# LabJunBMI/E3-invaraint-diffusion-model

Measured on AMD Instinct MI355X. Metric: denoising-steps/sec (batched pocket graphs), higher is better.
Workload: dtype f32 storage and accumulation, f16x3 products (fp32 grade); 1 GPU; structure_model sampling step, 256 x 256-residue pockets per GPU, 12+12 layers x 768, T=1000 schedule, encoder recomputed every step (as the reference); pockets_per_gpu=256, seq_len=256, parallelism=pocket-sharded x1, no collective

## Files before the change

### e3-invaraint-diffusion-model_amd/csrc/gemm_split.hip

```cpp
#include <type_traits>

#include "e3d_common.h"

namespace {

typedef __bf16 bf16x8 __attribute__((ext_vector_type(8)));
typedef __bf16 bf16x4 __attribute__((ext_vector_type(4)));
typedef _Float16 f16x8 __attribute__((ext_vector_type(8)));
typedef _Float16 f16x4 __attribute__((ext_vector_type(4)));

template <typename E> struct Vec;
template <> struct Vec<__bf16> { typedef bf16x8 x8; typedef bf16x4 x4; };
template <> struct Vec<_Float16> { typedef f16x8 x8; typedef f16x4 x4; };
__device__ __forceinline__ f32x16 mma16(const bf16x8 a, const bf16x8 b, const f32x16 c) {
    return __builtin_amdgcn_mfma_f32_32x32x16_bf16(a, b, c, 0, 0, 0);
}
__device__ __forceinline__ f32x16 mma16(const f16x8 a, const f16x8 b, const f32x16 c) {
    return __builtin_amdgcn_mfma_f32_32x32x16_f16(a, b, c, 0, 0, 0);
}

struct Epi { float* absmax; float scale; };

constexpr int BN = 128, BK = 32;
#ifdef GEMM_STAMPS
// ... 681 lines not shown
#pragma unroll
    for (int m = 0; m < 4; ++m) {
#pragma unroll
        for (int n = 0; n < 2; ++n) {
            const int col = col0 + wc * 64 + n * 32 + l31;
            const float bv = bias ? bias[col] : 0.f;
#pragma unroll
            for (int r = 0; r < 16; ++r) {
                const int row = row0 + wr * 128 + m * 32 + mfma32_row(r, half);
                float v = fmaf(acc[m][n][r], out_scale, bv);
                if (ACT == E3D_ACT_GELU) v = gelu_erf(v);
                if (ACT == E3D_ACT_SILU) v = silu(v);
                if (row < M) {
                    out[(int64_t)row * ldc + col] = v;
                    if (ACT == E3D_ACT_NONE && absmax) e3d_absmax_accum(amax, v);
                }
            }
        }
    }
    if (ACT == E3D_ACT_NONE && absmax) e3d_absmax_commit(amax, absmax, lane);
    STAMP_K(4);
#ifdef E3D_STAMPS
    asm volatile("s_waitcnt vmcnt(0)" ::: "memory");
    STAMP_K(5);
#endif
}

#ifdef E3D_NT_STORES
#define E3D_STORE_OUT(ptr, val) __builtin_nontemporal_store((val), (ptr))
#else
#define E3D_STORE_OUT(ptr, val) (*(ptr) = (val))
#endif

template <int ACT, typename E>
__global__ __launch_bounds__(512, 2) void gemm_split256p_kernel(const float* __restrict__ A, int64_t lda,
                                                                 const float* __restrict__ W,
                                                                 const float* __restrict__ bias,
                                                                 float* __restrict__ out, int64_t ldc, int N, int K,
                                                                 int tiles_m, int tiles_n, float* __restrict__ absmax, float out_scale) {
    extern __shared__ __attribute__((aligned(16))) unsigned char smem_raw[];
    constexpr int NS = 2, T_BYTES = BT * ROW64, BUF_BYTES = 2 * NS * T_BYTES;
    constexpr int NI = 8;
    const int total = tiles_m * tiles_n, nk = K / BK;
    const int tid = threadIdx.x, lane = tid & 63, wid = tid >> 6;
    const int wr = wid >> 2, wc = wid & 3;
    const int l31 = lane & 31, half = lane >> 5;

    unsigned goff[NI];
    int dst[NI];
#pragma unroll
    for (int i = 0; i < NI; ++i) {
        const int f = tid + 512 * (i & 3), r = f >> 3, kg = f & 7;
        goff[i] = (unsigned)(r * (i < 4 ? (int)lda : K) + kg * 4);
        dst[i] = (i < 4 ? 0 : NS * T_BYTES) + swz_off(r, kg >> 1) + (kg & 1) * 8;
    }

    int ld_tile = blockIdx.x, ld_k = 0;
    const float* ld_a;
    const float* ld_w;
    auto cursor_bases = [&]() {
        const int lid = xcd_remap(ld_tile, total);
        ld_a = A + (int64_t)(lid / tiles_n) * BT * lda + ld_k * BK;
        ld_w = W + (int64_t)(lid % tiles_n) * BT * K + ld_k * BK;
    };
    auto cursor_advance = [&]() {
        if (ld_k + 1 < nk) {
            ++ld_k;
            ld_a += BK;
            ld_w += BK;
        } else if (ld_tile + (int)gridDim.x < total) {
            ld_tile += gridDim.x;
            ld_k = 0;
            cursor_bases();
        }
    };
    f32x4 rg[NI];
    auto item_load = [&](int i) { rg[i] = *reinterpret_cast<const f32x4*>((i < 4 ? ld_a : ld_w) + goff[i]); };
    auto item_store = [&](int i, unsigned char* buf) {
        typename Vec<E>::x4 p[NS];
        split4<NS, E>(rg[i], p);
#pragma unroll
        for (int s = 0; s < NS; ++s) *reinterpret_cast<typename Vec<E>::x4*>(buf + s * T_BYTES + dst[i]) = p[s];
    };
    cursor_bases();
#pragma unroll
    for (int i = 0; i < NI; ++i) item_load(i);
    cursor_advance();
#pragma unroll
    for (int i = 0; i < NI; ++i) item_store(i, smem_raw);
#pragma unroll
    for (int i = 0; i < NI; ++i) item_load(i);
    cursor_advance();
    __syncthreads();

    int a_row[4], b_row[2];
#pragma unroll
    for (int m = 0; m < 4; ++m) a_row[m] = wr * 128 + m * 32 + l31;
#pragma unroll
    for (int n = 0; n < 2; ++n) b_row[n] = wc * 64 + n * 32 + l31;
    int cur = 0;
    unsigned amax = 0;

    for (int tile = blockIdx.x; tile < total; tile += gridDim.x) {
        f32x16 acc[4][2];
#pragma unroll
        for (int m = 0; m < 4; ++m)
#pragma unroll
            for (int n = 0; n < 2; ++n)
#pragma unroll
                for (int r = 0; r < 16; ++r) acc[m][n][r] = 0.f;
        for (int kt = 0; kt < nk; ++kt) {
            const unsigned char* base = smem_raw + cur * BUF_BYTES;
            unsigned char* next = smem_raw + (cur ^ 1) * BUF_BYTES;
#pragma unroll
            for (int ks = 0; ks < 2; ++ks) {
                typename Vec<E>::x8 fa[NS][4], fb[NS][2];
#pragma unroll
                for (int s = 0; s < NS; ++s) {
#pragma unroll
                    for (int n = 0; n < 2; ++n)
                        fb[s][n] = *reinterpret_cast<const typename Vec<E>::x8*>(base + (NS + s) * T_BYTES +
                                                                    swz_off(b_row[n], 2 * ks + half));
#pragma unroll
                    for (int m = 0; m < 4; ++m)
                        fa[s][m] = *reinterpret_cast<const typename Vec<E>::x8*>(base + s * T_BYTES + swz_off(a_row[m], 2 * ks + half));
                }
#pragma unroll
                for (int m = 0; m < 4; ++m) {
                    const int g = ks * 4 + m;
                    item_store(g, next);
                    item_load(g);
#pragma unroll
                    for (int n = 0; n < 2; ++n) {
                        acc[m][n] = mma16(fa[0][m], fb[1][n], acc[m][n]);
                        acc[m][n] = mma16(fa[1][m], fb[0][n], acc[m][n]);
                        acc[m][n] = mma16(fa[0][m], fb[0][n], acc[m][n]);
                    }
                    __builtin_amdgcn_sched_barrier(0);
                }
            }
            cursor_advance();
            __syncthreads();
            cur ^= 1;
        }

        const int lid = xcd_remap(tile, total);
        const int row0 = (lid / tiles_n) * BT, col0 = (lid % tiles_n) * BT;
#pragma unroll
        for (int m = 0; m < 4; ++m) {
#pragma unroll
            for (int n = 0; n < 2; ++n) {
                const int col = col0 + wc * 64 + n * 32 + l31;
                const float bv = bias ? bias[col] : 0.f;
                float* o = out + (int64_t)(row0 + wr * 128 + m * 32 + 4 * half) * ldc + col;
#pragma unroll
                for (int r = 0; r < 16; ++r) {
                    float v = fmaf(acc[m][n][r], out_scale, bv);
                    if (ACT == E3D_ACT_GELU) v = gelu_erf(v);
                    if (ACT == E3D_ACT_SILU) v = silu(v);
                    E3D_STORE_OUT(&o[(int64_t)((r & 3) + 8 * (r >> 2)) * ldc], v);
                    if (ACT == E3D_ACT_NONE && absmax) e3d_absmax_accum(amax, v);
                }
            }
        }
    }
    if (ACT == E3D_ACT_NONE && absmax) e3d_absmax_commit(amax, absmax, lane);
}

template <int ACT, typename E>
int launch256p(const float* A, int64_t lda, const float* W, const float* bias, float* out, int64_t ldc, int M, int N,
               int K, Epi epi, hipStream_t s) {
    const int tiles_m = M / BT, tiles_n = N / BT;
    constexpr size_t lds = 2 * 2 * 2 * BT * ROW64;
    static std::atomic<uint64_t> lds_ok{0};
    const int n_cu = e3d_cu_count();
    const int total = tiles_m * tiles_n;
    e3d_allow_lds(lds_ok, gemm_split256p_kernel<ACT, E>, lds);
    hipLaunchKernelGGL((gemm_split256p_kernel<ACT, E>), dim3(total < n_cu ? total : n_cu), dim3(512), lds, s, A, lda, W, bias, out,
                       ldc, N, K, tiles_m, tiles_n, epi.absmax, epi.scale);
    return e3d_launch_status("e3d_gemm_f32_split (persistent 256x256)");
}

int g_general_form = -1;
int g_tile_pref = -1;

template <int NS, int ACT, int WR, int WC, int NBUF, bool PIPE, typename E>
int launch256(const float* A, int64_t lda, const float* W, const float* bias, float* out, int64_t ldc, int M, int N,
              int K, Epi epi, hipStream_t s) {
    constexpr int TM = WR * 128, TN = WC * 64;
    const int tiles_m = (M + TM - 1) / TM, tiles_n = N / TN;
    const size_t lds = (size_t)NBUF * NS * (TM + TN) * ROW64;
    static std::atomic<uint64_t> lds_ok{0};
    e3d_allow_lds(lds_ok, gemm_split256_kernel<NS, ACT, WR, WC, NBUF, PIPE, E>, lds);
    hipLaunchKernelGGL((gemm_split256_kernel<NS, ACT, WR, WC, NBUF, PIPE, E>), dim3(tiles_m * tiles_n), dim3(WR * WC * 64), lds, s,
                       A, lda, W, bias, out, ldc, M, N, K, tiles_m, tiles_n, epi.absmax, epi.scale);
    return e3d_launch_status("e3d_gemm_f32_split (128x64 wave tiles)");
}

template <int NS, int ACT, bool A_KMAJ, bool B_KMAJ, int WM, int WN, typename E, int TN = 2, bool TR = false>
int launch_general(const float* A, int64_t lda, const float* B, int64_t ldb, const float* bias, float* out, int64_t ldc,
                   int M, int N, int K, Epi epi, hipStream_t s);

int p_min() {
    static int v = 0;
    if (!v) {
        const char* e = getenv("E3D_GEMM_P_MIN");
        v = e ? atoi(e) : 160;
    }
    return v;
}

template <int NS, int ACT, bool A_KMAJ, bool B_KMAJ, typename E>
int launch(const float* A, int64_t lda, const float* B, int64_t ldb, const float* bias, float* out, int64_t ldc,
           int M, int N, int K, Epi epi, hipStream_t s) {
    if (g_tile_pref < 0) {
        const char* e = getenv("E3D_GEMM_TILE");
        g_tile_pref = e ? atoi(e) : 4;
// ... 86 lines not shown
    return e3d_launch_status("e3d_gemm_f32_split");
}

template <int NS, typename E>
int dispatch(int act, bool a_kmaj, bool b_kmaj, const float* A, int64_t lda, const float* B, int64_t ldb,
             const float* bias, float* out, int64_t ldc, int M, int N, int K, Epi epi, hipStream_t s) {
    if (!a_kmaj && !b_kmaj) {
        switch (act) {
            case E3D_ACT_NONE: return launch<NS, E3D_ACT_NONE, false, false, E>(A, lda, B, ldb, bias, out, ldc, M, N, K, epi, s);
            case E3D_ACT_GELU: return launch<NS, E3D_ACT_GELU, false, false, E>(A, lda, B, ldb, bias, out, ldc, M, N, K, epi, s);
            case E3D_ACT_SILU: return launch<NS, E3D_ACT_SILU, false, false, E>(A, lda, B, ldb, bias, out, ldc, M, N, K, epi, s);
        }
        e3d_set_error("gemm_split: unknown activation %d", act);
        return -1;
    }
    if (act != E3D_ACT_NONE) {
        e3d_set_error("gemm_split: activations are only fused for the forward (K-contiguous) layout");
        return -1;
    }
    if (!a_kmaj && b_kmaj) return launch<NS, E3D_ACT_NONE, false, true, __bf16>(A, lda, B, ldb, bias, out, ldc, M, N, K, epi, s);
    if (a_kmaj && b_kmaj) return launch<NS, E3D_ACT_NONE, true, true, __bf16>(A, lda, B, ldb, bias, out, ldc, M, N, K, Epi{nullptr, epi.scale}, s);
    return launch<NS, E3D_ACT_NONE, true, false, __bf16>(A, lda, B, ldb, bias, out, ldc, M, N, K, epi, s);
}

}

#ifdef GEMM_STAMPS
extern "C" int e3d_debug_gemm_stamps(long long* t) { return (int)hipMemcpyFromSymbol(t, HIP_SYMBOL(gemm_stamps), sizeof(long long) * 2 * 64 * 8); }
#endif

#ifdef E3D_STAMPS
extern "C" int e3d_debug_read_stamps(long long* host_out) {
    return (int)hipMemcpyFromSymbol(host_out, HIP_SYMBOL(e3d_stamps), sizeof(long long) * 2 * 32 * 8);
}
#endif

extern "C" int e3d_gemm_kernel_select(int pref) {
    if (g_tile_pref < 0) {
        const char* e = getenv("E3D_GEMM_TILE");
        g_tile_pref = e ? atoi(e) : 4;
    }
    const int prev = g_tile_pref;
    if (pref >= 0) g_tile_pref = pref;
    return prev;
}

extern "C" int e3d_gemm_general_select(int form) {
    if (g_general_form < 0) {
        const char* e = getenv("E3D_GEMM_FORM");
        g_general_form = e ? atoi(e) : 0;
    }
    const int prev = g_general_form;
    if (form >= 0) g_general_form = form;
    return prev;
}

static int gemm_split_general(const float* A, int64_t lda, int a_kmajor, const float* B, int64_t ldb, int b_kmajor,
                              const float* bias, float* out, int64_t ldc, int M, int N, int K, int act, int terms,
                              float* absmax, float out_scale, void* stream) {
    const Epi epi{absmax, out_scale};
    E3D_REQUIRE(out_scale == 1.0f || !(a_kmajor && b_kmajor), "gemm_split: out_scale is not available for the split-K layout");
    E3D_REQUIRE(A && B && out, "gemm_split: null pointer");
    E3D_REQUIRE(M > 0 && N > 0 && K > 0, "gemm_split: bad shape M=%d N=%d K=%d", M, N, K);
    E3D_REQUIRE(terms == E3D_TERMS_BF16 || terms == 3 || terms == 6 || terms == E3D_TERMS_F16X3,
                "gemm_split: terms must be 1, 3, 6 or 19 (got %d)", terms);
    E3D_REQUIRE(ldc >= N, "gemm_split: ldc=%lld < N=%d", (long long)ldc, N);
// ... 134 lines not shown
```

### e3-invaraint-diffusion-model_amd/csrc/gemm_rowln.hip

```cpp
#include <type_traits>

#include "e3d_common.h"

namespace {

typedef __bf16 bf16x8 __attribute__((ext_vector_type(8)));
typedef _Float16 f16x8 __attribute__((ext_vector_type(8)));
template <typename E> struct V8;
template <> struct V8<__bf16> { typedef bf16x8 t; };
template <> struct V8<_Float16> { typedef f16x8 t; };
__device__ __forceinline__ f32x16 mma16(const bf16x8 a, const bf16x8 b, const f32x16 c) {
    return __builtin_amdgcn_mfma_f32_32x32x16_bf16(a, b, c, 0, 0, 0);
}
__device__ __forceinline__ f32x16 mma16(const f16x8 a, const f16x8 b, const f32x16 c) {
    return __builtin_amdgcn_mfma_f32_32x32x16_f16(a, b, c, 0, 0, 0);
}

constexpr int RN = 768, RBM = 96, NBLK = RN / 32;
constexpr int W_STEP = NBLK * 2 * 1024;
constexpr int A_PAIR = 128 * 128;
constexpr int LDS_A = 2 * W_STEP;
constexpr int RES_CHUNK = 16 * RN * 4;
constexpr int LDS_STATS = 3 * RES_CHUNK;
constexpr int LDS_COLS = LDS_STATS + (8 * RBM + RBM) * 4;
// ... 27 lines not shown
    const int piece = blockIdx.x * 4 + (threadIdx.x >> 6);
    const int nblk = N / 32;
    if (piece >= (K / 16) * nblk) return;
    const int ks = piece / nblk, nb = piece % nblk;
    const float* src = W + (int64_t)(nb * 32 + (lane & 31)) * K + ks * 16 + 8 * (lane >> 5);
    const f32x4 a = *reinterpret_cast<const f32x4*>(src), b = *reinterpret_cast<const f32x4*>(src + 4);
    typename V8<E>::t hi, lo;
    split8(a, b, hi, lo);
    unsigned char* dst = out + (int64_t)piece * 2048 + lane * 16;
    *reinterpret_cast<typename V8<E>::t*>(dst) = hi;
    *reinterpret_cast<typename V8<E>::t*>(dst + 1024) = lo;
}

#ifndef ROWLN_LAB
#define ROWLN_LAB 0
#endif
#ifdef ROWLN_STAMPS
__device__ long long rowln_stamps[2][64][8];
__device__ long long rowln_tile_stamps[2][8][8];
__device__ long long rowln_wg_times[512][4];
#define RSTAMP(step, slot)                                                                                        \
    do {                                                                                                          \
        if (stamp_on && (step) < 64 && lane == 0) rowln_stamps[wid >> 2][(step)][(slot)] = __builtin_readcyclecounter(); \
    } while (0)
#define TSTAMP(slot)                                                                                              \
    do {                                                                                                          \
        if (stamp_on && tile_no < 8 && lane == 0) rowln_tile_stamps[wid >> 2][tile_no][(slot)] = __builtin_readcyclecounter(); \
    } while (0)
#else
#define RSTAMP(step, slot) do {} while (0)
#define TSTAMP(slot) do {} while (0)
#endif
#define E3D_VMCNT(n) asm volatile("s_waitcnt vmcnt(" #n ")" ::: "memory")
#define E3D_BARRIER()                          \
    do {                                       \
        asm volatile("" ::: "memory");         \
        __builtin_amdgcn_s_barrier();          \
        asm volatile("" ::: "memory");         \
        __builtin_amdgcn_sched_barrier(0);     \
    } while (0)
#define E3D_LDS_BARRIER()                                   \
    do {                                                    \
        asm volatile("s_waitcnt lgkmcnt(0)" ::: "memory");  \
        E3D_BARRIER();                                      \
    } while (0)

template <int OFF = 0>
__device__ __forceinline__ void glds16(const void* g, unsigned char* lds_wave_base) {
    __builtin_amdgcn_global_load_lds((const __attribute__((address_space(1))) void*)g,
                                     (__attribute__((address_space(3))) void*)lds_wave_base, 16, OFF, 0);
}

__device__ __forceinline__ int next_tile_rows(int left, int pattern, int group_rows) {
#ifndef ROWLN_NO_PATTERNS
    if (group_rows == 256) {
        if (pattern == 1 && left == 256) return 64;
        if (pattern == 2 && left == 160) return 64;
        if (pattern == 3) return 64;
    }
#endif
    if (left >= 160 || left == 96) return 96;
    if (left > 96) return 64;
    return left;
}

template <typename E>
__global__ __launch_bounds__(512, 2) void gemm_rowln_kernel(const float* __restrict__ A, int64_t lda,
                                                            const unsigned char* __restrict__ Wp, const float* __restrict__ bias,
                                                            const float* __restrict__ res, int64_t ldr,
                                                            const float* __restrict__ gamma, const float* __restrict__ beta,
                                                            float eps, float* __restrict__ out, int64_t ldo, int M, int K,
                                                            int rows_per_wg, float out_scale) {
    extern __shared__ __attribute__((aligned(16))) unsigned char smem[];
    typedef typename V8<E>::t X8;
    const int tid = threadIdx.x, lane = tid & 63;
    const int wid = __builtin_amdgcn_readfirstlane(tid >> 6);
    const int l31 = lane & 31, half = lane >> 5;
    const int npairs = K / 32, last_step = 2 * npairs - 1;

    int row0 = blockIdx.x * rows_per_wg;
    const int row_end = min(M, row0 + rows_per_wg);
    if (row0 >= row_end) return;

    const unsigned w_lane = (unsigned)(wid * 6144 + lane * 16);
    unsigned a_lane[2];
    auto a_offsets = [&](int rows) {
#pragma unroll
        for (int i = 0; i < 2; ++i) {
            const int row = (wid + 8 * i) * 8 + (lane >> 3);
            a_lane[i] = (unsigned)(min(row, rows - 1) * (int)lda + (((lane & 7) ^ ((row >> 1) & 7)) << 2)) * 4u;
        }
    };
    unsigned r_lane[2];
#pragma unroll
    for (int j = 0; j < 2; ++j) r_lane[j] = (unsigned)((2 * wid + j) * (int)ldr + lane * 4) * 4u;
    const int a_roff = LDS_A + l31 * 128 + (((2 * half) ^ ((l31 >> 1) & 7)) << 4);
    const int b_roff = (wid * 3) * 2048 + lane * 16;

    auto issue_w = [&](int src, int buf) {
        const unsigned char* g = Wp + (int64_t)src * W_STEP + w_lane;
        unsigned char* l = smem + buf * W_STEP + wid * 6144;
        glds16<0>(g, l);
        glds16<1024>(g, l);
        glds16<2048>(g, l);
        glds16<3072>(g, l);
        glds16<0>(g + 4096, l + 4096);
        glds16<1024>(g + 4096, l + 4096);
    };
    auto issue_a = [&](const float* a_tile, int pair, int buf) {
        const unsigned char* g = reinterpret_cast<const unsigned char*>(a_tile + pair * 32);
        unsigned char* l = smem + LDS_A + buf * A_PAIR + wid * 1024;
        glds16<0>(g + a_lane[0], l);
        glds16<0>(g + a_lane[1], l + 8192);
    };

    float* red = reinterpret_cast<float*>(smem + LDS_STATS);
    float* rowc = red + 8 * RBM;
    const int colbase = wid * 96 + l31;
    float* colc = reinterpret_cast<float*>(smem + LDS_COLS);
    for (int i = tid; i < RN; i += 512) {
        colc[i] = bias ? bias[i] : 0.f;
        colc[RN + i] = gamma[i];
        colc[2 * RN + i] = beta[i];
    }
    asm volatile("s_waitcnt vmcnt(0) lgkmcnt(0)" ::: "memory");
    constexpr float inv_n = 1.0f / RN;
    const bool bit8 = (lane & 8) != 0, bit4 = (lane & 4) != 0, bit2 = (lane & 2) != 0,
               bit1 = (lane & 1) != 0;

    const int pattern = (blockIdx.x >> 3) & 3, group_rows = row_end - row0;
    int rows = next_tile_rows(row_end - row0, pattern, group_rows);
    a_offsets(rows);
    issue_a(A + (int64_t)row0 * lda, 0, 0);
    issue_w(0, 0);
    issue_w(1, 1);
    issue_a(A + (int64_t)row0 * lda, 1, 1);
    int next_row0 = 0, next_rows = 0;
#ifdef ROWLN_STAMPS
    const bool stamp_on = blockIdx.x == 77 && (wid & 3) == 0;
    int tile_no = 0;
    if (tid == 0 && blockIdx.x < 512) {
        rowln_wg_times[blockIdx.x][0] = __builtin_amdgcn_s_memrealtime();
        rowln_wg_times[blockIdx.x][1] = __builtin_readcyclecounter();
    }
#endif

    auto tile_body = [&](auto nm_c) -> bool {
        constexpr int NM = decltype(nm_c)::value;
        const float* a_tile = A + (int64_t)row0 * lda;
        f32x16 acc[NM][3];
#pragma unroll
        for (int m = 0; m < NM; ++m)
#pragma unroll
            for (int n = 0; n < 3; ++n)
#pragma unroll
                for (int r = 0; r < 16; ++r) acc[m][n][r] = 0.f;

        TSTAMP(0);
        int a_cur = 0, a_nxt = A_PAIR, a_nx2 = 2 * A_PAIR;
        E3D_VMCNT(8);
        E3D_BARRIER();
// ... 61 lines not shown
                    E3D_VMCNT(8);
                    RSTAMP(stamp_step, 3);
                    const unsigned char* wn = smem + (KS ^ 1) * W_STEP + b_roff;
#pragma unroll
                    for (int n = 0; n < 3; ++n) {
                        nh[n] = *reinterpret_cast<const X8*>(wn + n * 2048);
                        nl[n] = *reinterpret_cast<const X8*>(wn + n * 2048 + 1024);
                    }
                    const int an = KS == 0 ? a_cur : a_nxt;
                    y0 = *reinterpret_cast<const f32x4*>(smem + an + (a_roff ^ (64 * (KS ^ 1))));
                    y1 = *reinterpret_cast<const f32x4*>(smem + an + (a_roff ^ (64 * (KS ^ 1) + 16)));
                    __builtin_amdgcn_sched_barrier(0);
                }
            }
            x0 = y0;
            x1 = y1;
            RSTAMP(stamp_step, 2);
        };

        for (int p = 0; p < npairs; ++p) {
            const bool last_pair = p + 1 == npairs;
            step(std::integral_constant<int, 0>{}, bh0, bl0, bh1, bl1, min(2 * p + 2, last_step), 0, last_pair && res_on ? 0 : -1, 2 * p);
            step(std::integral_constant<int, 1>{}, bh1, bl1, bh0, bl0, min(2 * p + 3, last_step), last_pair ? -1 : min(p + 2, npairs - 1),
                 last_pair && res_on ? 1 : -1, 2 * p + 1);
            const int t = a_cur;
            a_cur = a_nxt;
            a_nxt = a_nx2;
            a_nx2 = t;
        }
        if (!res_on) E3D_VMCNT(0);
        E3D_LDS_BARRIER();
        TSTAMP(2);

#pragma unroll
        for (int m = 0; m < NM; ++m)
#pragma unroll
            for (int n = 0; n < 3; ++n)
#pragma unroll
                for (int r = 0; r < 16; ++r) acc[m][n][r] = fmaf(acc[m][n][r], out_scale, colc[colbase + 32 * n]);
        if (res_on) {
            auto issue_r = [&](int c) {
                const unsigned char* g = res_tile + c * res_chunk_stride;
                unsigned char* l = smem + (c % 3) * RES_CHUNK + wid * 6144;
                glds16<0>(g + r_lane[0], l);
                glds16<1024>(g + r_lane[0], l);
                glds16<2048>(g + r_lane[0], l);
                glds16<0>(g + r_lane[1], l + 3072);
                glds16<1024>(g + r_lane[1], l + 3072);
                glds16<2048>(g + r_lane[1], l + 3072);
            };
            constexpr int NCH = 2 * NM;
#pragma unroll
            for (int c = 0; c < NCH; ++c) {
                if (c + 1 < NCH) E3D_VMCNT(6);
                else E3D_VMCNT(0);
                E3D_BARRIER();
                if (c + 2 < NCH) issue_r(c + 2);
                const int m = c >> 1, r0 = 8 * (c & 1);
                const unsigned char* cb = smem + (c % 3) * RES_CHUNK + colbase * 4 + half * (4 * RN * 4);
#pragma unroll
                for (int n = 0; n < 3; ++n)
#pragma unroll
                    for (int j = 0; j < 8; ++j) {
                        const int lr = (j & 3) + 8 * (j >> 2);
                        acc[m][n][r0 + j] += *reinterpret_cast<const float*>(cb + lr * (RN * 4) + n * 128);
                    }
            }
        }
        E3D_LDS_BARRIER();
        TSTAMP(3);

        next_row0 = row0 + 32 * NM;
        const bool more = next_row0 < row_end;
        if (more) {
            next_rows = next_tile_rows(row_end - next_row0, pattern, group_rows);
            a_offsets(next_rows);
            issue_a(A + (int64_t)next_row0 * lda, 0, 0);
            issue_w(0, 0);
            issue_w(1, 1);
            issue_a(A + (int64_t)next_row0 * lda, 1, 1);
        }

        if (ROWLN_LAB & 16) {
#pragma unroll
            for (int m = 0; m < NM; ++m)
#pragma unroll
                for (int n = 0; n < 3; ++n) asm volatile("" :: "v"(acc[m][n]));
            if (more) E3D_LDS_BARRIER();
            return more;
        }
        auto swap16_sum = [&](float lo, float hi) -> float {
            const auto r = __builtin_amdgcn_permlane16_swap(__float_as_uint(lo), __float_as_uint(hi), false, false);
            return __uint_as_float(r[0]) + __uint_as_float(r[1]);
        };
        auto dpp_xchg = [&](float lo, float hi, bool up, auto ctrl_c) -> float {
            constexpr int CTRL = decltype(ctrl_c)::value;
            const float send = up ? lo : hi, keep = up ? hi : lo;
            return keep + __uint_as_float(__builtin_amdgcn_update_dpp(0u, __float_as_uint(send), CTRL, 0xF, 0xF, true));
        };
        constexpr int ROW_MIRROR = 0x140, ROW_HALF_MIRROR = 0x141, QUAD_XOR2 = 0x4E, QUAD_XOR1 = 0xB1;
        auto reduce_in_row = [&](float (&w)[16]) -> float {
#pragma unroll
            for (int j = 0; j < 8; ++j) w[j] = dpp_xchg(w[j], w[j + 8], bit8, std::integral_constant<int, ROW_MIRROR>{});
#pragma unroll
            for (int j = 0; j < 4; ++j) w[j] = dpp_xchg(w[j], w[j + 4], bit4, std::integral_constant<int, ROW_HALF_MIRROR>{});
#pragma unroll
            for (int j = 0; j < 2; ++j) w[j] = dpp_xchg(w[j], w[j + 2], bit2, std::integral_constant<int, QUAD_XOR2>{});
            return dpp_xchg(w[0], w[1], bit1, std::integral_constant<int, QUAD_XOR1>{});
        };
        auto reduce32 = [&](float (&v)[32]) -> float {
            float w[16];
#pragma unroll
            for (int j = 0; j < 16; ++j) w[j] = swap16_sum(v[j], v[j + 16]);
            return reduce_in_row(w);
        };
        auto reduce16 = [&](float (&u)[16]) -> float {
            float w[16];
#pragma unroll
            for (int j = 0; j < 16; ++j) w[j] = swap16_sum(u[j], u[j]);
            return reduce_in_row(w);
        };
        constexpr bool PAIR = NM >= 2, SINGLE = NM != 2;
        constexpr int MS = NM - 1;
        const int row_v = 32 * (l31 >> 4) + mfma32_row(l31 & 15, half), row_u = 32 * MS + mfma32_row(l31 & 15, half);
        auto exchange = [&](float tv, float tu, bool variance) {
            if (PAIR) red[wid * RBM + row_v] = tv;
            if (SINGLE && l31 < 16) red[wid * RBM + row_u] = tu;
            E3D_LDS_BARRIER();
            if (tid < 32 * NM) {
                const float t = ((red[tid] + red[RBM + tid]) + (red[2 * RBM + tid] + red[3 * RBM + tid])) +
                                ((red[4 * RBM + tid] + red[5 * RBM + tid]) + (red[6 * RBM + tid] + red[7 * RBM + tid]));
                rowc[tid] = variance ? 1.0f / sqrtf(t * inv_n + eps) : t * inv_n;
            }
            E3D_LDS_BARRIER();
        };
        {
            float v[32], u[16], tv = 0.f, tu = 0.f;
#pragma unroll
            for (int m = 0; m < NM; ++m)
#pragma unroll
                for (int r = 0; r < 16; ++r) {
                    const float t = (acc[m][0][r] + acc[m][1][r]) + acc[m][2][r];
                    if (PAIR && m < 2) v[m * 16 + r] = t;
                    else u[r] = t;
                }
            if (PAIR) tv = reduce32(v);
            if (SINGLE) tu = reduce16(u);
            exchange(tv, tu, false);
        }
        {
            float v[32], u[16], tv = 0.f, tu = 0.f;
#pragma unroll
            for (int m = 0; m < NM; ++m)
#pragma unroll
                for (int q = 0; q < 4; ++q) {
                    const f32x4 mean = *reinterpret_cast<const f32x4*>(rowc + m * 32 + 8 * q + 4 * half);
#pragma unroll
                    for (int j = 0; j < 4; ++j) {
                        float t = 0.f;
#pragma unroll
                        for (int n = 0; n < 3; ++n) {
                            const float d = acc[m][n][4 * q + j] - mean[j];
                            acc[m][n][4 * q + j] = d;
                            t = fmaf(d, d, t);
                        }
                        if (PAIR && m < 2) v[m * 16 + 4 * q + j] = t;
                        else u[4 * q + j] = t;
                    }
                }
            if (PAIR) tv = reduce32(v);
            if (SINGLE) tu = reduce16(u);
            exchange(tv, tu, true);
        }
        TSTAMP(4);
        float gv[3], bt[3];
#pragma unroll
        for (int n = 0; n < 3; ++n) {
            gv[n] = colc[RN + colbase + 32 * n];
            bt[n] = colc[2 * RN + colbase + 32 * n];
        }
#pragma unroll
        for (int m = 0; m < NM; ++m)
#pragma unroll
            for (int q = 0; q < 4; ++q) {
                const f32x4 rstd = *reinterpret_cast<const f32x4*>(rowc + m * 32 + 8 * q + 4 * half);
                float* o = out + (int64_t)(row0 + m * 32 + 8 * q + 4 * half) * ldo + colbase;
#pragma unroll
                for (int j = 0; j < 4; ++j)
#pragma unroll
                    for (int n = 0; n < 3; ++n) o[(int64_t)j * ldo + 32 * n] = fmaf(acc[m][n][4 * q + j] * rstd[j], gv[n], bt[n]);
            }
        TSTAMP(5);
#ifdef ROWLN_STAMPS
        asm volatile("s_waitcnt vmcnt(0)" ::: "memory");
        TSTAMP(6);
        ++tile_no;
#endif
        if (more) E3D_LDS_BARRIER();
        return more;
    };

    while (true) {
        bool more;
        if (rows == 96) more = tile_body(std::integral_constant<int, 3>{});
        else if (rows == 64) more = tile_body(std::integral_constant<int, 2>{});
        else more = tile_body(std::integral_constant<int, 1>{});
        if (!more) break;
        row0 = next_row0;
        rows = next_rows;
    }
    E3D_VMCNT(0);
#ifdef ROWLN_STAMPS
    if (tid == 0 && blockIdx.x < 512) {
        rowln_wg_times[blockIdx.x][2] = __builtin_amdgcn_s_memrealtime();
        rowln_wg_times[blockIdx.x][3] = __builtin_readcyclecounter();
    }
#endif
}

template <typename E>
int launch_rowln(const float* A, int64_t lda, const void* Wp, const float* bias, const float* res, int64_t ldr,
                 const float* gamma, const float* beta, float eps, float* out, int64_t ldo, int M, int K, float out_scale,
                 hipStream_t s) {
    static std::atomic<uint64_t> lds_ok{0};
    e3d_allow_lds(lds_ok, gemm_rowln_kernel<E>, (size_t)LDS_TOTAL);
    const int n_cu = e3d_cu_count();
    const int rows_per_wg = ((M + n_cu - 1) / n_cu + 31) / 32 * 32;
    const int grid = (M + rows_per_wg - 1) / rows_per_wg;
    hipLaunchKernelGGL((gemm_rowln_kernel<E>), dim3(grid), dim3(512), LDS_TOTAL, s, A, lda,
                       reinterpret_cast<const unsigned char*>(Wp), bias, res, ldr, gamma, beta, eps, out, ldo, M, K, rows_per_wg,
                       out_scale);
// ... 50 lines not shown
```

Baseline: 3889 pocket-steps/s.

## Stagger persistent GEMM work by splitting first tile into half units on alternate CUs

Measured after the change: 3844 pocket-steps/s (median of 2 runs). 0.989x the previous value.

```diff
diff --git a/e3-invaraint-diffusion-model_amd/csrc/gemm_split.hip b/e3-invaraint-diffusion-model_amd/csrc/gemm_split.hip
--- a/e3-invaraint-diffusion-model_amd/csrc/gemm_split.hip
+++ b/e3-invaraint-diffusion-model_amd/csrc/gemm_split.hip
@@ -737,12 +737,23 @@
 #define E3D_STORE_OUT(ptr, val) (*(ptr) = (val))
 #endif
 
+#ifdef E3D_STAMPS
+__device__ long long e3d_pstamps[256][16][6];
+#define PSTAMP(u, slot, val)                                                                          \
+    do {                                                                                              \
+        if (tid == 0 && blockIdx.x < 256 && (u) < 16) e3d_pstamps[blockIdx.x][(u)][(slot)] = (val);   \
+    } while (0)
+#else
+#define PSTAMP(u, slot, val) do {} while (0)
+#endif
+
 template <int ACT, typename E>
 __global__ __launch_bounds__(512, 2) void gemm_split256p_kernel(const float* __restrict__ A, int64_t lda,
                                                                  const float* __restrict__ W,
                                                                  const float* __restrict__ bias,
                                                                  float* __restrict__ out, int64_t ldc, int N, int K,
-                                                                 int tiles_m, int tiles_n, float* __restrict__ absmax, float out_scale) {
+                                                                 int tiles_m, int tiles_n, float* __restrict__ absmax, float out_scale,
+                                                                 int stagger) {
     extern __shared__ __attribute__((aligned(16))) unsigned char smem_raw[];
     constexpr int NS = 2, T_BYTES = BT * ROW64, BUF_BYTES = 2 * NS * T_BYTES;
     constexpr int NI = 8;
@@ -760,12 +771,20 @@
         dst[i] = (i < 4 ? 0 : NS * T_BYTES) + swz_off(r, kg >> 1) + (kg & 1) * 8;
     }
 
-    int ld_tile = blockIdx.x, ld_k = 0;
+    const int G = gridDim.x, n_tiles = (total - (int)blockIdx.x + G - 1) / G;
+    const bool stag = stagger && ((blockIdx.x >> 3) & 1);
+    const int units = n_tiles + (stag ? 1 : 0);
+    auto unit_tile = [&](int u) { return (int)blockIdx.x + G * (stag && u == units - 1 ? 0 : u); };
+    auto unit_half = [&](int u) { return !stag ? -1 : (u == 0 ? 0 : (u == units - 1 ? 1 : -1)); };
+
+    int ld_u = 0, ld_k = 0;
+    bool ld_half = false;
     const float* ld_a;
     const float* ld_w;
     auto cursor_bases = [&]() {
-        const int lid = xcd_remap(ld_tile, total);
-        ld_a = A + (int64_t)(lid / tiles_n) * BT * lda + ld_k * BK;
+        const int lid = xcd_remap(unit_tile(ld_u), total), h = unit_half(ld_u);
+        ld_half = h >= 0;
+        ld_a = A + ((int64_t)(lid / tiles_n) * BT + (h > 0 ? BT / 2 : 0)) * lda + ld_k * BK;
         ld_w = W + (int64_t)(lid % tiles_n) * BT * K + ld_k * BK;
     };
     auto cursor_advance = [&]() {
@@ -773,13 +792,14 @@
             ++ld_k;
             ld_a += BK;
             ld_w += BK;
-        } else if (ld_tile + (int)gridDim.x < total) {
-            ld_tile += gridDim.x;
+        } else if (ld_u + 1 < units) {
+            ++ld_u;
             ld_k = 0;
             cursor_bases();
         }
     };
     f32x4 rg[NI];
+    bool rg_half = false;
     auto item_load = [&](int i) { rg[i] = *reinterpret_cast<const f32x4*>((i < 4 ? ld_a : ld_w) + goff[i]); };
     auto item_store = [&](int i, unsigned char* buf) {
         typename Vec<E>::x4 p[NS];
@@ -787,39 +807,44 @@
 #pragma unroll
         for (int s = 0; s < NS; ++s) *reinterpret_cast<typename Vec<E>::x4*>(buf + s * T_BYTES + dst[i]) = p[s];
     };
+    auto stage = [&](int g, unsigned char* buf, bool st_half, bool ld_h) {
+        if ((g != 2 && g != 3) || !st_half) item_store(g, buf);
+        if ((g != 2 && g != 3) || !ld_h) item_load(g);
+    };
     cursor_bases();
 #pragma unroll
-    for (int i = 0; i < NI; ++i) item_load(i);
+    for (int i = 0; i < NI; ++i)
+        if ((i != 2 && i != 3) || !ld_half) item_load(i);
+    rg_half = ld_half;
     cursor_advance();
 #pragma unroll
-    for (int i = 0; i < NI; ++i) item_store(i, smem_raw);
-#pragma unroll
-    for (int i = 0; i < NI; ++i) item_load(i);
+    for (int i = 0; i < NI; ++i)
+        if ((i != 2 && i != 3) || !rg_half) item_store(i, smem_raw);
+#pragma unroll
+    for (int i = 0; i < NI; ++i)
+        if ((i != 2 && i != 3) || !ld_half) item_load(i);
+    rg_half = ld_half;
     cursor_advance();
     __syncthreads();
 
-    int a_row[4], b_row[2];
-#pragma unroll
-    for (int m = 0; m < 4; ++m) a_row[m] = wr * 128 + m * 32 + l31;
-#pragma unroll
-    for (int n = 0; n < 2; ++n) b_row[n] = wc * 64 + n * 32 + l31;
     int cur = 0;
     unsigned amax = 0;
-
-    for (int tile = blockIdx.x; tile < total; tile += gridDim.x) {
-        f32x16 acc[4][2];
-#pragma unroll
-        for (int m = 0; m < 4; ++m)
-#pragma unroll
-            for (int n = 0; n < 2; ++n)
-#pragma unroll
-                for (int r = 0; r < 16; ++r) acc[m][n][r] = 0.f;
+    f32x16 acc[4][2];
+
+    auto k_loop = [&](auto mh_tag, int u) {
+        constexpr int MH = decltype(mh_tag)::value;
+        int a_row[MH], b_row[2];
+#pragma unroll
+        for (int m = 0; m < MH; ++m) a_row[m] = wr * (32 * MH) + m * 32 + l31;
+#pragma unroll
+        for (int n = 0; n < 2; ++n) b_row[n] = wc * 64 + n * 32 + l31;
         for (int kt = 0; kt < nk; ++kt) {
             const unsigned char* base = smem_raw + cur * BUF_BYTES;
             unsigned char* next = smem_raw + (cur ^ 1) * BUF_BYTES;
+            const bool st_half = rg_half, ld_h = ld_half;
 #pragma unroll
             for (int ks = 0; ks < 2; ++ks) {
-                typename Vec<E>::x8 fa[NS][4], fb[NS][2];
+                typename Vec<E>::x8 fa[NS][MH], fb[NS][2];
 #pragma unroll
                 for (int s = 0; s < NS; ++s) {
 #pragma unroll
@@ -827,16 +852,20 @@
                         fb[s][n] = *reinterpret_cast<const typename Vec<E>::x8*>(base + (NS + s) * T_BYTES +
                                                                     swz_off(b_row[n], 2 * ks + half));
 #pragma unroll
-                    for (int m = 0; m < 4; ++m)
+                    for (int m = 0; m < MH; ++m)
                         fa[s][m] = *reinterpret_cast<const typename Vec<E>::x8*>(base + s * T_BYTES + swz_off(a_row[m], 2 * ks + half));
                 }
 #pragma unroll
-                for (int m = 0; m < 4; ++m) {
-                    const int g = ks * 4 + m;
-                    item_store(g, next);
-                    item_load(g);
+                for (int q = 0; q < 4; ++q) {
+                    const int g = ks * 4 + q;
+                    stage(g, next, st_half, ld_h);
+#ifdef E3D_STAMPS
+                    if (kt == 0 && g == 0) PSTAMP(u, 2, (long long)__builtin_readcyclecounter());
+#endif
 #pragma unroll
                     for (int n = 0; n < 2; ++n) {
+                        if (MH == 2 && n != (q & 1)) continue;
+                        const int m = MH == 4 ? q : q >> 1;
                         acc[m][n] = mma16(fa[0][m], fb[1][n], acc[m][n]);
                         acc[m][n] = mma16(fa[1][m], fb[0][n], acc[m][n]);
                         acc[m][n] = mma16(fa[0][m], fb[0][n], acc[m][n]);
@@ -844,20 +873,23 @@
                     __builtin_amdgcn_sched_barrier(0);
                 }
             }
+            rg_half = ld_h;
             cursor_advance();
             __syncthreads();
             cur ^= 1;
         }
-
-        const int lid = xcd_remap(tile, total);
-        const int row0 = (lid / tiles_n) * BT, col0 = (lid % tiles_n) * BT;
-#pragma unroll
-        for (int m = 0; m < 4; ++m) {
+    };
+    auto epilogue = [&](auto mh_tag, int u) {
+        constexpr int MH = decltype(mh_tag)::value;
+        const int lid = xcd_remap(unit_tile(u), total), h = unit_half(u);
+        const int row0 = (lid / tiles_n) * BT + (h > 0 ? BT / 2 : 0), col0 = (lid % tiles_n) * BT;
+#pragma unroll
+        for (int m = 0; m < MH; ++m) {
 #pragma unroll
             for (int n = 0; n < 2; ++n) {
                 const int col = col0 + wc * 64 + n * 32 + l31;
                 const float bv = bias ? bias[col] : 0.f;
-                float* o = out + (int64_t)(row0 + wr * 128 + m * 32 + 4 * half) * ldc + col;
+                float* o = out + (int64_t)(row0 + wr * (32 * MH) + m * 32 + 4 * half) * ldc + col;
 #pragma unroll
                 for (int r = 0; r < 16; ++r) {
                     float v = fmaf(acc[m][n][r], out_scale, bv);
@@ -868,9 +900,34 @@
                 }
             }
         }
+    };
+
+    for (int u = 0; u < units; ++u) {
+        PSTAMP(u, 0, (long long)__builtin_amdgcn_s_memrealtime());
+#pragma unroll
+        for (int m = 0; m < 4; ++m)
+#pragma unroll
+            for (int n = 0; n < 2; ++n)
+#pragma unroll
+                for (int r = 0; r < 16; ++r) acc[m][n][r] = 0.f;
+        const bool whole = unit_half(u) < 0;
+        if (whole) k_loop(std::integral_constant<int, 4>(), u);
+        else k_loop(std::integral_constant<int, 2>(), u);
+        PSTAMP(u, 1, (long long)__builtin_amdgcn_s_memrealtime());
+        PSTAMP(u, 3, (long long)__builtin_readcyclecounter());
+        if (whole) epilogue(std::integral_constant<int, 4>(), u);
+        else epilogue(std::integral_constant<int, 2>(), u);
+        PSTAMP(u, 4, (long long)__builtin_readcyclecounter());
     }
     if (ACT == E3D_ACT_NONE && absmax) e3d_absmax_commit(amax, absmax, lane);
-}
+#ifdef E3D_STAMPS
+    asm volatile("s_waitcnt vmcnt(0)" ::: "memory");
+    PSTAMP(units - 1, 5, (long long)__builtin_readcyclecounter());
+#endif
+}
+
+int g_general_form = -1;
+int g_tile_pref = -1;
 
 template <int ACT, typename E>
 int launch256p(const float* A, int64_t lda, const float* W, const float* bias, float* out, int64_t ldc, int M, int N,
@@ -880,14 +937,13 @@
     static std::atomic<uint64_t> lds_ok{0};
     const int n_cu = e3d_cu_count();
     const int total = tiles_m * tiles_n;
+    const int stagger = g_tile_pref != 6 && total >= 2 * n_cu && total % n_cu == 0;
     e3d_allow_lds(lds_ok, gemm_split256p_kernel<ACT, E>, lds);
     hipLaunchKernelGGL((gemm_split256p_kernel<ACT, E>), dim3(total < n_cu ? total : n_cu), dim3(512), lds, s, A, lda, W, bias, out,
-                       ldc, N, K, tiles_m, tiles_n, epi.absmax, epi.scale);
+                       ldc, N, K, tiles_m, tiles_n, epi.absmax, epi.scale, stagger);
     return e3d_launch_status("e3d_gemm_f32_split (persistent 256x256)");
 }
 
-int g_general_form = -1;
-int g_tile_pref = -1;
 
 template <int NS, int ACT, int WR, int WC, int NBUF, bool PIPE, typename E>
 int launch256(const float* A, int64_t lda, const float* W, const float* bias, float* out, int64_t ldc, int M, int N,
@@ -1040,6 +1096,13 @@
 #ifdef E3D_STAMPS
 extern "C" int e3d_debug_read_stamps(long long* host_out) {
     return (int)hipMemcpyFromSymbol(host_out, HIP_SYMBOL(e3d_stamps), sizeof(long long) * 2 * 32 * 8);
+}
+extern "C" int e3d_debug_read_pstamps(long long* host_out) {
+    return (int)hipMemcpyFromSymbol(host_out, HIP_SYMBOL(e3d_pstamps), sizeof(long long) * 256 * 16 * 6);
+}
+extern "C" int e3d_debug_clear_pstamps() {
+    static long long zero[256 * 16 * 6];
+    return (int)hipMemcpyToSymbol(HIP_SYMBOL(e3d_pstamps), zero, sizeof(zero));
 }
 #endif
 
```

## Pipeline row-LayerNorm epilogue per 16-row chunk, overlapping residual DMA and stats

Applied to the files above, without the earlier changes.

Result: no change. 3924 pocket-steps/s before, 3930 pocket-steps/s after, median of 6 (+0.2%).

```diff
diff --git a/e3-invaraint-diffusion-model_amd/csrc/gemm_rowln.hip b/e3-invaraint-diffusion-model_amd/csrc/gemm_rowln.hip
--- a/e3-invaraint-diffusion-model_amd/csrc/gemm_rowln.hip
+++ b/e3-invaraint-diffusion-model_amd/csrc/gemm_rowln.hip
@@ -83,6 +83,25 @@
 #define TSTAMP(slot) do {} while (0)
 #endif
 #define E3D_VMCNT(n) asm volatile("s_waitcnt vmcnt(" #n ")" ::: "memory")
+template <int N>
+__device__ __forceinline__ void vmcnt_wait() {
+    static_assert(N >= 0 && N < 64, "vmcnt is a 6-bit count");
+    asm volatile("s_waitcnt vmcnt(%0)" :: "n"(N) : "memory");
+}
+template <typename T>
+__device__ __forceinline__ T fresh(T x) {
+    asm volatile("" : "+v"(x));
+    return x;
+}
+template <int I, int N, typename F>
+__device__ __forceinline__ void static_for(F&& f) {
+    if constexpr (I < N) {
+        f(std::integral_constant<int, I>{});
+        static_for<I + 1, N>(f);
+    }
+}
+constexpr int epi_dma(int s, int nch) { return s + 2 < nch ? 6 : 0; }
+constexpr int epi_stores(int s, int nch, bool ln) { return ln && s >= 4 && s - 4 < nch ? 24 : 0; }
 #define E3D_BARRIER()                          \
     do {                                       \
         asm volatile("" ::: "memory");         \
@@ -136,10 +155,11 @@
     const unsigned w_lane = (unsigned)(wid * 6144 + lane * 16);
     unsigned a_lane[2];
     auto a_offsets = [&](int rows) {
+        const int ln = fresh(lane);
 #pragma unroll
         for (int i = 0; i < 2; ++i) {
-            const int row = (wid + 8 * i) * 8 + (lane >> 3);
-            a_lane[i] = (unsigned)(min(row, rows - 1) * (int)lda + (((lane & 7) ^ ((row >> 1) & 7)) << 2)) * 4u;
+            const int row = (wid + 8 * i) * 8 + (ln >> 3);
+            a_lane[i] = (unsigned)(min(row, rows - 1) * (int)lda + (((ln & 7) ^ ((row >> 1) & 7)) << 2)) * 4u;
         }
     };
     unsigned r_lane[2];
@@ -149,7 +169,7 @@
     const int b_roff = (wid * 3) * 2048 + lane * 16;
 
     auto issue_w = [&](int src, int buf) {
-        const unsigned char* g = Wp + (int64_t)src * W_STEP + w_lane;
+        const unsigned char* g = Wp + (int64_t)src * W_STEP + fresh(w_lane);
         unsigned char* l = smem + buf * W_STEP + wid * 6144;
         glds16<0>(g, l);
         glds16<1024>(g, l);
@@ -166,7 +186,6 @@
     };
 
     float* red = reinterpret_cast<float*>(smem + LDS_STATS);
-    float* rowc = red + 8 * RBM;
     const int colbase = wid * 96 + l31;
     float* colc = reinterpret_cast<float*>(smem + LDS_COLS);
     for (int i = tid; i < RN; i += 512) {
@@ -176,8 +195,7 @@
     }
     asm volatile("s_waitcnt vmcnt(0) lgkmcnt(0)" ::: "memory");
     constexpr float inv_n = 1.0f / RN;
-    const bool bit8 = (lane & 8) != 0, bit4 = (lane & 4) != 0, bit2 = (lane & 2) != 0,
-               bit1 = (lane & 1) != 0;
+    const bool bit8 = (lane & 8) != 0, bit4 = (lane & 4) != 0;
 
     const int pattern = (blockIdx.x >> 3) & 3, group_rows = row_end - row0;
     int rows = next_tile_rows(row_end - row0, pattern, group_rows);
@@ -305,63 +323,21 @@
         E3D_LDS_BARRIER();
         TSTAMP(2);
 
-#pragma unroll
-        for (int m = 0; m < NM; ++m)
-#pragma unroll
-            for (int n = 0; n < 3; ++n)
-#pragma unroll
-                for (int r = 0; r < 16; ++r) acc[m][n][r] = fmaf(acc[m][n][r], out_scale, colc[colbase + 32 * n]);
-        if (res_on) {
-            auto issue_r = [&](int c) {
-                const unsigned char* g = res_tile + c * res_chunk_stride;
-                unsigned char* l = smem + (c % 3) * RES_CHUNK + wid * 6144;
-                glds16<0>(g + r_lane[0], l);
-                glds16<1024>(g + r_lane[0], l);
-                glds16<2048>(g + r_lane[0], l);
-                glds16<0>(g + r_lane[1], l + 3072);
-                glds16<1024>(g + r_lane[1], l + 3072);
-                glds16<2048>(g + r_lane[1], l + 3072);
-            };
-            constexpr int NCH = 2 * NM;
-#pragma unroll
-            for (int c = 0; c < NCH; ++c) {
-                if (c + 1 < NCH) E3D_VMCNT(6);
-                else E3D_VMCNT(0);
-                E3D_BARRIER();
-                if (c + 2 < NCH) issue_r(c + 2);
-                const int m = c >> 1, r0 = 8 * (c & 1);
-                const unsigned char* cb = smem + (c % 3) * RES_CHUNK + colbase * 4 + half * (4 * RN * 4);
-#pragma unroll
-                for (int n = 0; n < 3; ++n)
-#pragma unroll
-                    for (int j = 0; j < 8; ++j) {
-                        const int lr = (j & 3) + 8 * (j >> 2);
-                        acc[m][n][r0 + j] += *reinterpret_cast<const float*>(cb + lr * (RN * 4) + n * 128);
-                    }
-            }
-        }
-        E3D_LDS_BARRIER();
-        TSTAMP(3);
-
+        constexpr int NCH = 2 * NM;
+        constexpr bool LN = !(ROWLN_LAB & 16);
         next_row0 = row0 + 32 * NM;
         const bool more = next_row0 < row_end;
-        if (more) {
-            next_rows = next_tile_rows(row_end - next_row0, pattern, group_rows);
-            a_offsets(next_rows);
-            issue_a(A + (int64_t)next_row0 * lda, 0, 0);
-            issue_w(0, 0);
-            issue_w(1, 1);
-            issue_a(A + (int64_t)next_row0 * lda, 1, 1);
-        }
-
-        if (ROWLN_LAB & 16) {
-#pragma unroll
-            for (int m = 0; m < NM; ++m)
-#pragma unroll
-                for (int n = 0; n < 3; ++n) asm volatile("" :: "v"(acc[m][n]));
-            if (more) E3D_LDS_BARRIER();
-            return more;
-        }
+        auto issue_r = [&](int c) {
+            const unsigned char* g = res_tile + c * res_chunk_stride;
+            unsigned char* l = smem + (c % 3) * RES_CHUNK + wid * 6144;
+            glds16<0>(g + r_lane[0], l);
+            glds16<1024>(g + r_lane[0], l);
+            glds16<2048>(g + r_lane[0], l);
+            glds16<0>(g + r_lane[1], l + 3072);
+            glds16<1024>(g + r_lane[1], l + 3072);
+            glds16<2048>(g + r_lane[1], l + 3072);
+        };
+
         auto swap16_sum = [&](float lo, float hi) -> float {
             const auto r = __builtin_amdgcn_permlane16_swap(__float_as_uint(lo), __float_as_uint(hi), false, false);
             return __uint_as_float(r[0]) + __uint_as_float(r[1]);
@@ -371,105 +347,136 @@
             const float send = up ? lo : hi, keep = up ? hi : lo;
             return keep + __uint_as_float(__builtin_amdgcn_update_dpp(0u, __float_as_uint(send), CTRL, 0xF, 0xF, true));
         };
+        auto dpp_add = [&](float x, auto ctrl_c) -> float {
+            constexpr int CTRL = decltype(ctrl_c)::value;
+            return x + __uint_as_float(__builtin_amdgcn_update_dpp(0u, __float_as_uint(x), CTRL, 0xF, 0xF, true));
+        };
         constexpr int ROW_MIRROR = 0x140, ROW_HALF_MIRROR = 0x141, QUAD_XOR2 = 0x4E, QUAD_XOR1 = 0xB1;
-        auto reduce_in_row = [&](float (&w)[16]) -> float {
-#pragma unroll
-            for (int j = 0; j < 8; ++j) w[j] = dpp_xchg(w[j], w[j + 8], bit8, std::integral_constant<int, ROW_MIRROR>{});
-#pragma unroll
-            for (int j = 0; j < 4; ++j) w[j] = dpp_xchg(w[j], w[j + 4], bit4, std::integral_constant<int, ROW_HALF_MIRROR>{});
-#pragma unroll
-            for (int j = 0; j < 2; ++j) w[j] = dpp_xchg(w[j], w[j + 2], bit2, std::integral_constant<int, QUAD_XOR2>{});
-            return dpp_xchg(w[0], w[1], bit1, std::integral_constant<int, QUAD_XOR1>{});
-        };
-        auto reduce32 = [&](float (&v)[32]) -> float {
-            float w[16];
-#pragma unroll
-            for (int j = 0; j < 16; ++j) w[j] = swap16_sum(v[j], v[j + 16]);
-            return reduce_in_row(w);
-        };
-        auto reduce16 = [&](float (&u)[16]) -> float {
-            float w[16];
-#pragma unroll
-            for (int j = 0; j < 16; ++j) w[j] = swap16_sum(u[j], u[j]);
-            return reduce_in_row(w);
-        };
-        constexpr bool PAIR = NM >= 2, SINGLE = NM != 2;
-        constexpr int MS = NM - 1;
-        const int row_v = 32 * (l31 >> 4) + mfma32_row(l31 & 15, half), row_u = 32 * MS + mfma32_row(l31 & 15, half);
-        auto exchange = [&](float tv, float tu, bool variance) {
-            if (PAIR) red[wid * RBM + row_v] = tv;
-            if (SINGLE && l31 < 16) red[wid * RBM + row_u] = tu;
+        auto reduce8 = [&](float (&v)[8]) -> float {
+            float w[4];
+#pragma unroll
+            for (int j = 0; j < 4; ++j) w[j] = swap16_sum(v[j], v[j + 4]);
+#pragma unroll
+            for (int j = 0; j < 2; ++j) w[j] = dpp_xchg(w[j], w[j + 2], bit8, std::integral_constant<int, ROW_MIRROR>{});
+            const float x = dpp_xchg(w[0], w[1], bit4, std::integral_constant<int, ROW_HALF_MIRROR>{});
+            return dpp_add(dpp_add(x, std::integral_constant<int, QUAD_XOR2>{}), std::integral_constant<int, QUAD_XOR1>{});
+        };
+        float* part = red;
+        float* rowc = red + 2 * 2 * 8 * 16;
+        const int prow = ((lane >> 2) & 3) + 8 * ((lane >> 4) & 1) + 4 * half;
+        auto publish = [&](int pass, int c, float x) {
+            if ((lane & 3) == 0) part[(pass * 2 + (c & 1)) * 128 + fresh(wid * 16 + prow)] = x;
+        };
+
+        static_for<0, NCH + 4>([&](auto t_c) {
+            constexpr int t = decltype(t_c)::value;
+            if constexpr (t < NCH) {
+                if (res_on) vmcnt_wait<epi_stores(t - 2, NCH, LN) + epi_dma(t - 1, NCH) + epi_stores(t - 1, NCH, LN)>();
+            }
             E3D_LDS_BARRIER();
-            if (tid < 32 * NM) {
-                const float t = ((red[tid] + red[RBM + tid]) + (red[2 * RBM + tid] + red[3 * RBM + tid])) +
-                                ((red[4 * RBM + tid] + red[5 * RBM + tid]) + (red[6 * RBM + tid] + red[7 * RBM + tid]));
-                rowc[tid] = variance ? 1.0f / sqrtf(t * inv_n + eps) : t * inv_n;
-            }
-            E3D_LDS_BARRIER();
-        };
-        {
-            float v[32], u[16], tv = 0.f, tu = 0.f;
+            if constexpr (t == NCH) {
+                if (more) {
+                    next_rows = next_tile_rows(row_end - next_row0, pattern, group_rows);
+                    a_offsets(next_rows);
+                    issue_a(A + (int64_t)next_row0 * lda, 0, 0);
+                    issue_w(0, 0);
+                    issue_w(1, 1);
+                    issue_a(A + (int64_t)next_row0 * lda, 1, 1);
+                }
+            }
+            if constexpr (t + 2 < NCH) {
+                if (res_on) issue_r(t + 2);
+            }
+            asm volatile("" ::: "memory");
+            __builtin_amdgcn_sched_barrier(0);
+            if constexpr (LN && t >= 1 && t - 3 < NCH) {
+                if (wid == 0 && lane < 32) {
+                    const int l = fresh(lane), pass = l >> 4, c = t - 1 - 2 * pass;
+                    if (c >= 0 && c < NCH) {
+                        const float* p = part + (pass * 2 + (c & 1)) * 128 + (l & 15);
+                        const float s = ((p[0] + p[16]) + (p[32] + p[48])) + ((p[64] + p[80]) + (p[96] + p[112]));
+                        rowc[(pass * 2 + (c & 1)) * 16 + (l & 15)] = pass ? 1.0f / sqrtf(fmaf(s, inv_n, eps)) : s * inv_n;
+                    }
+                }
+            }
+            if constexpr (t < NCH) {
+                constexpr int m = t >> 1, r0 = 8 * (t & 1);
+#pragma unroll
+                for (int n = 0; n < 3; ++n) {
+                    const float bs = colc[colbase + 32 * n];
+#pragma unroll
+                    for (int j = 0; j < 8; ++j) acc[m][n][r0 + j] = fmaf(acc[m][n][r0 + j], out_scale, bs);
+                }
+                if (res_on) {
+                    const unsigned char* cb = smem + (t % 3) * RES_CHUNK + fresh(colbase * 4 + half * (4 * RN * 4));
+#pragma unroll
+                    for (int n = 0; n < 3; ++n)
+#pragma unroll
+                        for (int j = 0; j < 8; ++j) {
+                            const int lr = (j & 3) + 8 * (j >> 2);
+                            acc[m][n][r0 + j] += *reinterpret_cast<const float*>(cb + lr * (RN * 4) + n * 128);
+                        }
+                }
+                if constexpr (LN) {
+                    float v[8];
+#pragma unroll
+                    for (int j = 0; j < 8; ++j) v[j] = (acc[m][0][r0 + j] + acc[m][1][r0 + j]) + acc[m][2][r0 + j];
+                    publish(0, t, reduce8(v));
+                }
+                if constexpr (t == NCH - 1) TSTAMP(3);
+            }
+            if constexpr (LN && t >= 2 && t - 2 < NCH) {
+                constexpr int c = t - 2, m = c >> 1, r0 = 8 * (c & 1);
+                const float* mp = rowc + (c & 1) * 16 + fresh(4 * half);
+                const f32x4 mlo = *reinterpret_cast<const f32x4*>(mp), mhi = *reinterpret_cast<const f32x4*>(mp + 8);
+                float v[8];
+#pragma unroll
+                for (int j = 0; j < 8; ++j) {
+                    const float mean = j < 4 ? mlo[j] : mhi[j - 4];
+                    float s = 0.f;
+#pragma unroll
+                    for (int n = 0; n < 3; ++n) {
+                        const float d = acc[m][n][r0 + j] - mean;
+                        acc[m][n][r0 + j] = d;
+                        s = fmaf(d, d, s);
+                    }
+                    v[j] = s;
+                }
+                publish(1, c, reduce8(v));
+            }
+            if constexpr (LN && t >= 4) {
+                constexpr int c = t - 4, m = c >> 1, r0 = 8 * (c & 1);
+                const float* rp = rowc + (2 + (c & 1)) * 16 + fresh(4 * half);
+                const f32x4 slo = *reinterpret_cast<const f32x4*>(rp), shi = *reinterpret_cast<const f32x4*>(rp + 8);
+                float gv[3], bt[3];
+#pragma unroll
+                for (int n = 0; n < 3; ++n) {
+                    gv[n] = colc[RN + colbase + 32 * n];
+                    bt[n] = colc[2 * RN + colbase + 32 * n];
+                }
+                float* o = out + (int64_t)(row0 + 16 * c + 4 * half) * ldo + colbase;
+#pragma unroll
+                for (int j = 0; j < 8; ++j) {
+                    const float rstd = j < 4 ? slo[j] : shi[j - 4];
+#pragma unroll
+                    for (int n = 0; n < 3; ++n)
+                        o[(int64_t)((j & 3) + 8 * (j >> 2)) * ldo + 32 * n] = fmaf(acc[m][n][r0 + j] * rstd, gv[n], bt[n]);
+                }
+            }
+            if constexpr (t == NCH + 2) TSTAMP(4);
+        });
+        if (!LN) {
 #pragma unroll
             for (int m = 0; m < NM; ++m)
 #pragma unroll
-                for (int r = 0; r < 16; ++r) {
-                    const float t = (acc[m][0][r] + acc[m][1][r]) + acc[m][2][r];
-                    if (PAIR && m < 2) v[m * 16 + r] = t;
-                    else u[r] = t;
-                }
-            if (PAIR) tv = reduce32(v);
-            if (SINGLE) tu = reduce16(u);
-            exchange(tv, tu, false);
+                for (int n = 0; n < 3; ++n) asm volatile("" :: "v"(acc[m][n]));
         }
-        {
-            float v[32], u[16], tv = 0.f, tu = 0.f;
-#pragma unroll
-            for (int m = 0; m < NM; ++m)
-#pragma unroll
-                for (int q = 0; q < 4; ++q) {
-                    const f32x4 mean = *reinterpret_cast<const f32x4*>(rowc + m * 32 + 8 * q + 4 * half);
-#pragma unroll
-                    for (int j = 0; j < 4; ++j) {
-                        float t = 0.f;
-#pragma unroll
-                        for (int n = 0; n < 3; ++n) {
-                            const float d = acc[m][n][4 * q + j] - mean[j];
-                            acc[m][n][4 * q + j] = d;
-                            t = fmaf(d, d, t);
-                        }
-                        if (PAIR && m < 2) v[m * 16 + 4 * q + j] = t;
-                        else u[4 * q + j] = t;
-                    }
-                }
-            if (PAIR) tv = reduce32(v);
-            if (SINGLE) tu = reduce16(u);
-            exchange(tv, tu, true);
-        }
-        TSTAMP(4);
-        float gv[3], bt[3];
-#pragma unroll
-        for (int n = 0; n < 3; ++n) {
-            gv[n] = colc[RN + colbase + 32 * n];
-            bt[n] = colc[2 * RN + colbase + 32 * n];
-        }
-#pragma unroll
-        for (int m = 0; m < NM; ++m)
-#pragma unroll
-            for (int q = 0; q < 4; ++q) {
-                const f32x4 rstd = *reinterpret_cast<const f32x4*>(rowc + m * 32 + 8 * q + 4 * half);
-                float* o = out + (int64_t)(row0 + m * 32 + 8 * q + 4 * half) * ldo + colbase;
-#pragma unroll
-                for (int j = 0; j < 4; ++j)
-#pragma unroll
-                    for (int n = 0; n < 3; ++n) o[(int64_t)j * ldo + 32 * n] = fmaf(acc[m][n][4 * q + j] * rstd[j], gv[n], bt[n]);
-            }
         TSTAMP(5);
 #ifdef ROWLN_STAMPS
         asm volatile("s_waitcnt vmcnt(0)" ::: "memory");
         TSTAMP(6);
         ++tile_no;
 #endif
-        if (more) E3D_LDS_BARRIER();
         return more;
     };
 
```
